# jinhojsk515/spmm

Hardware: AMD Instinct MI355X
Metric: pretrain molecules/sec (higher is better)
Workload: dtype bf16; 1 GPU; SPMM pretrain step, text 12 layers (fusion at 6) + PV 6 layers, H=768, 12 heads, queue 36864, train mode (dropout 0.1), fwd+bwd+clip+AdamW+EMA; global_batch=128, seq_len=128, parallelism=dp1, schedule=eager launches on three HIP streams, packed text rows

## Files before the change

include/spmm_hip.h:

```cpp
#ifndef SPMM_HIP_H
#define SPMM_HIP_H

#include <stdint.h>

#ifdef __HIPCC__
#include <hip/hip_runtime.h>
typedef hipStream_t spmm_stream_t;
#else
typedef void* spmm_stream_t;
#endif

#ifdef __cplusplus
extern "C" {
#endif

int spmm_version(void);
const char* spmm_last_error(void);

#define SPMM_EPI_BF16 0
#define SPMM_EPI_GELU 1
#define SPMM_EPI_F32 2
#define SPMM_EPI_F32_ATOMIC 3
#define SPMM_EPI_GELU_GRAD 4
#define SPMM_EPI_F32_ACC 5
#define SPMM_EPI_GELU_DERIV 6
#define SPMM_EPI_MUL 7

#define SPMM_GEMM_AUTO 0
#define SPMM_GEMM_K128 1
#define SPMM_GEMM_K256x128 2
#define SPMM_GEMM_K256 3
#define SPMM_GEMM_K128PC 5
#define SPMM_GEMM_K256P8 8
#define SPMM_GEMM_K256P8_TILES 9
#define SPMM_GEMM_AUTO_TILES 16
int spmm_gemm_nt(const void* A, long lda, const void* W, long ldw, int M, int N, int K, int splits, const float* bias,
                 const float* div_ptr, float alpha, const void* R, long ldr, const void* G, long ldg, void* C, long ldc,
                 void* C2, long ldc2, int epi, float* colsum, int kernel, const int* M_dev, spmm_stream_t stream);
long spmm_gemm_tn_workspace_bytes(int M, int N, int K, int splits);
int spmm_gemm_tn_splits(int M, int N, int K, int kernel);
int spmm_gemm_tn(const void* A, long lda, const void* B, long ldb, int M, int N, int K, int splits, float alpha, float* C,
                 long ldc, float* workspace, int kernel, const int* M_dev, spmm_stream_t stream);
int spmm_gemm_tn_reduce(const float* ws, int ns, int N, int K, float* C, long ldc, spmm_stream_t stream);
int spmm_colsum_bf16(const void* x, long ld, int R, int C, float* out, const int* R_dev, spmm_stream_t stream);

int spmm_attn_fwd(const void* Q, long ldq, const void* K, long ldk, const void* V, long ldv, const int* kmask,
                  const int* kv_seq, const int* q_row0, const int* q_len, const int* kv_row0, const int* kv_len, void* O,
                  long ldo, float* LSE, int nseq, int nH, int Lq, int Lkv, int causal_from, int is_cross, float dropout_p,
                  const uint64_t* seed_ptr, uint64_t seed_salt, int q_off, int kv_off, spmm_stream_t stream);
// ... 161 lines not shown
```

spmm_amd/csrc/gemm.hip:

```cpp
#include "common.h"
#include "../../include/spmm_hip.h"

namespace {

constexpr int BM = 128, BN = 128, BK = 64;
constexpr int TILE_BYTES = BM * BK * 2;
constexpr int STAGE_BYTES = 2 * TILE_BYTES;

enum Epi { EPI_BF16 = 0, EPI_GELU = 1, EPI_F32 = 2, EPI_F32_ATOMIC = 3, EPI_GELU_GRAD = 4, EPI_F32_ACC = 5, EPI_GELU_DERIV = 6, EPI_MUL = 7 };
constexpr bool epi_is_bf16(int e) { return e == EPI_BF16 || e == EPI_GELU || e == EPI_GELU_GRAD || e == EPI_GELU_DERIV || e == EPI_MUL; }

struct GemmP {
  const bf16* A; long lda;
  const bf16* W; long ldw;
  int M, N, K;
  int ksplit;
  const float* bias;
  const float* div_ptr;
  float alpha;
  const bf16* R; long ldr;
  const bf16* G; long ldg;
  void* C; long ldc;
  bf16* C2; long ldc2;
  float* colsum;
// ... 839 lines not shown
    if (p.colsum) {
#pragma unroll
      for (int e = 0; e < 8; ++e) {
        float t = cs[e];
        t += __shfl_xor(t, 8, 64);
        t += __shfl_xor(t, 16, 64);
        t += __shfl_xor(t, 32, 64);
        cs[e] = t;
      }
      if (lane < 8 && n_ok) {
#pragma unroll
        for (int e = 0; e < 8; ++e) atomicAdd(p.colsum + n + e, cs[e]);
      }
    }
  }
}

template <int EPI>
__global__ __launch_bounds__(512) void gemm_nt_p8_kernel(GemmP p) {
  extern __shared__ __attribute__((aligned(16))) char smem8[];
  const int tid = threadIdx.x, lane = tid & 63;
  const int wave = __builtin_amdgcn_readfirstlane(tid >> 6);
  const int wr = wave >> 2, wc = wave & 3;
  GEMM_DYN_M(p);
  const int ntm = (p.M + BM3 - 1) / BM3, ntn = (p.N + BN3 - 1) / BN3, nt = ntm * ntn;
  if ((int)blockIdx.x >= nt) return;
  const int nk = p.K / BK;

  f32x4 acc[2][4][4];
#define P8_ZERO()                                                              \
// ... 163 lines not shown
    P8_STAMP(2);

    if (wr == 0) P8_BAR();
    P8_SB();
    {
      int lane_e = lane;
      asm volatile("" : "+v"(lane_e));
      GemmP q = p;
      asm volatile("" : "+s"(q.C), "+s"(q.ldc), "+s"(q.C2), "+s"(q.ldc2));
      asm volatile("" : "+s"(q.R), "+s"(q.ldr), "+s"(q.G), "+s"(q.ldg));
      asm volatile("" : "+s"(q.bias), "+s"(q.colsum), "+s"(q.div_ptr), "+s"(q.alpha), "+s"(q.M), "+s"(q.N));
      auto hook = [](int) {};
      const uint32_t xb = lds0 + P8_LDS + wave * 4096;
      const int mb = cm0 + wr * 128, nb = cn0 + wc * 64;
      const bool interior = cm0 + BM3 <= q.M && cn0 + BN3 <= q.N;
      if constexpr (EPI == EPI_GELU_GRAD || EPI == EPI_MUL) {
        if (interior) p8_epilogue_blocks<EPI, true, true>(q, acc, xb, mb, nb, lane_e, hook);
        else p8_epilogue_blocks<EPI, false, true>(q, acc, xb, mb, nb, lane_e, hook);
      } else if (EPI == EPI_BF16 && q.R != nullptr) {
        if (interior) p8_epilogue_blocks<EPI, true, true>(q, acc, xb, mb, nb, lane_e, hook);
        else p8_epilogue_blocks<EPI, false, true>(q, acc, xb, mb, nb, lane_e, hook);
      } else {
        if (interior) p8_epilogue_blocks<EPI, true, false>(q, acc, xb, mb, nb, lane_e, hook);
        else p8_epilogue_blocks<EPI, false, false>(q, acc, xb, mb, nb, lane_e, hook);
      }
    }
    P8_SB();
    if (wr == 1) P8_BAR();
    P8_STAMP(4);
#ifdef P8_PROFILE
    ++prof_i;
// ... 20 lines not shown
#undef P8_LGKM0
}

template <typename K>
int raise_lds(K kernel, int bytes, const char* what) {
  hipError_t e = hipFuncSetAttribute((const void*)kernel, hipFuncAttributeMaxDynamicSharedMemorySize, bytes);
  if (e != hipSuccess) {
    spmm_set_error("spmm_gemm_nt: cannot raise the dynamic LDS of %s to %d: %s", what, bytes, hipGetErrorString(e));
    return SPMM_ERR_LAUNCH;
  }
  return SPMM_OK;
}

template <int EPI>
int launch_p8_one(const GemmP& p, hipStream_t st, bool persist) {
  static const int rc = raise_lds(gemm_nt_p8_kernel<EPI>, P8_LDS + P8_XLDS, "the 8-phase kernel");
  if (rc != SPMM_OK) return rc;
  const int nt = ((p.M + BM3 - 1) / BM3) * ((p.N + BN3 - 1) / BN3);
  static const int ncu = [] { int dev = 0, n = 0; (void)hipGetDevice(&dev); (void)hipDeviceGetAttribute(&n, hipDeviceAttributeMultiprocessorCount, dev); return n > 0 ? n & ~7 : 256; }();
  dim3 grid(persist && nt > ncu ? ncu : nt);
  hipLaunchKernelGGL((gemm_nt_p8_kernel<EPI>), grid, dim3(512), P8_LDS + P8_XLDS, st, p);
  return SPMM_OK;
}
int launch_p8(int epi, const GemmP& p, hipStream_t st, bool persist) {
  switch (epi) {
    case EPI_BF16: return launch_p8_one<EPI_BF16>(p, st, persist);
    case EPI_GELU: return launch_p8_one<EPI_GELU>(p, st, persist);
    case EPI_GELU_GRAD: return launch_p8_one<EPI_GELU_GRAD>(p, st, persist);
    case EPI_GELU_DERIV: return launch_p8_one<EPI_GELU_DERIV>(p, st, persist);
    case EPI_MUL: return launch_p8_one<EPI_MUL>(p, st, persist);
    default: return -1;
  }
}

template <int EPI>
int launch_v3_one(const GemmP& p, hipStream_t st) {
  static const int rc = raise_lds(gemm_nt_v3_kernel<EPI>, LDS3_BYTES, "the 256x256 kernel");
  if (rc != SPMM_OK) return rc;
  dim3 grid(((p.M + BM3 - 1) / BM3) * ((p.N + BN3 - 1) / BN3));
  hipLaunchKernelGGL((gemm_nt_v3_kernel<EPI>), grid, dim3(512), LDS3_BYTES, st, p);
  return SPMM_OK;
}
int launch_v3(int epi, const GemmP& p, hipStream_t st) {
  switch (epi) {
    case EPI_BF16: return launch_v3_one<EPI_BF16>(p, st);
// ... 51 lines not shown
    case EPI_BF16: hipLaunchKernelGGL((gemm_nt_kernel<EPI_BF16>), grid, dim3(256), 0, st, p); break;
    case EPI_GELU: hipLaunchKernelGGL((gemm_nt_kernel<EPI_GELU>), grid, dim3(256), 0, st, p); break;
    case EPI_F32: hipLaunchKernelGGL((gemm_nt_kernel<EPI_F32>), grid, dim3(256), 0, st, p); break;
    case EPI_F32_ATOMIC: hipLaunchKernelGGL((gemm_nt_kernel<EPI_F32_ATOMIC>), grid, dim3(256), 0, st, p); break;
    case EPI_GELU_GRAD: hipLaunchKernelGGL((gemm_nt_kernel<EPI_GELU_GRAD>), grid, dim3(256), 0, st, p); break;
    case EPI_F32_ACC: hipLaunchKernelGGL((gemm_nt_kernel<EPI_F32_ACC>), grid, dim3(256), 0, st, p); break;
    case EPI_GELU_DERIV: hipLaunchKernelGGL((gemm_nt_kernel<EPI_GELU_DERIV>), grid, dim3(256), 0, st, p); break;
    case EPI_MUL: hipLaunchKernelGGL((gemm_nt_kernel<EPI_MUL>), grid, dim3(256), 0, st, p); break;
    default: return -1;
  }
  return SPMM_OK;
}

inline bool is_bf16_epi(int epi) { return epi_is_bf16(epi); }
inline bool p8_ok(const GemmP& p, int epi) {
  return is_bf16_epi(epi) && p.K % 128 == 0 && p.N % 8 == 0 && (unsigned long)p.M * (unsigned long)p.lda * 2ul < (1ul << 32) &&
         (unsigned long)p.N * (unsigned long)p.ldw * 2ul < (1ul << 32);
}

int pick_tile(int M, int N, int epi) {
  const bool bf = is_bf16_epi(epi);
  if (M >= 6000) {
    const long t3 = (long)((M + 255) / 256) * ((N + 255) / 256);
    if (bf && t3 >= 96) return 3;
    return (epi != EPI_F32_ATOMIC) ? 2 : 1;
  }
  auto tiles = [&](int bm, int bn) { return (double)((M + bm - 1) / bm) * ((N + bn - 1) / bn); };
  auto fill = [](double t) { const double w = (double)(long)((t + 255) / 256); return t / (256.0 * w); };
  const double t3 = tiles(256, 256), t2 = tiles(256, 128), t1 = tiles(128, 128);
  const double s3 = bf ? 1.20 * fill(t3) : 0.0;
  const double s2 = (M >= 512 && epi != EPI_F32_ATOMIC) ? 0.85 * fill(t2) : 0.0;
  const double s1 = 0.80 * (t1 < 256 ? t1 / 256.0 : 1.0);
  if (s3 >= s2 && s3 >= s1) return 3;
  return s2 >= s1 ? 2 : 1;
}

}

extern "C" int spmm_gemm_nt(const void* A, long lda, const void* W, long ldw, int M, int N, int K, int splits,
// ... 13 lines not shown
  SPMM_CHECK_SHAPE(epi >= EPI_BF16 && epi <= EPI_MUL, "spmm_gemm_nt: unknown epilogue %d", epi);
  if (splits < 1) splits = 1;
  SPMM_CHECK_SHAPE(splits == 1 || epi == EPI_F32_ATOMIC, "spmm_gemm_nt: split-K needs the atomic epilogue");
  SPMM_CHECK_SHAPE((epi != EPI_GELU_GRAD && epi != EPI_MUL) || G != nullptr, "spmm_gemm_nt: the GELU-grad / multiply epilogues need G");
  SPMM_CHECK_SHAPE(colsum == nullptr || epi == EPI_BF16 || epi == EPI_GELU_GRAD || epi == EPI_MUL, "spmm_gemm_nt: colsum is only fused into the bf16 / GELU-grad / multiply epilogues");
  int ksplit = ((K / 64 + splits - 1) / splits) * 64;
  splits = (K + ksplit - 1) / ksplit;
  GemmP p;
  p.A = (const bf16*)A; p.lda = lda; p.W = (const bf16*)W; p.ldw = ldw;
  p.M = M; p.N = N; p.K = K; p.ksplit = ksplit; p.bias = bias; p.div_ptr = div_ptr; p.alpha = alpha;
  p.R = (const bf16*)R; p.ldr = ldr; p.G = (const bf16*)G; p.ldg = ldg; p.C = C; p.ldc = ldc;
  p.C2 = (bf16*)C2; p.ldc2 = ldc2; p.colsum = colsum;
  p.M_ptr = nullptr;
  p.order = K > 1024 ? 0 : 2;

  int k = kernel == SPMM_GEMM_AUTO_TILES ? 0 : kernel;
  if (k == 0) {
    const int tile = splits > 1 ? 1 : pick_tile(M, N, epi);
    k = tile == 3 ? (p8_ok(p, epi) ? (kernel == SPMM_GEMM_AUTO_TILES ? 9 : 8) : 3) : tile;
    if (k == 2 && (epi == EPI_F32_ATOMIC || M < 512)) k = 1;
  }
  const bool pc_fits = (unsigned long)p.M * (unsigned long)p.lda * 2ul < (1ul << 32) && (unsigned long)p.N * (unsigned long)p.ldw * 2ul < (1ul << 32);
  const long t128 = (long)((M + BM - 1) / BM) * ((N + BN - 1) / BN) * splits;
  if (k == 1 && kernel != 1 && pc_fits && PC_AUTO && t128 <= 256 && ksplit >= 4 * BK) k = 5;
  SPMM_CHECK_SHAPE(k == 1 || k == 2 || k == 3 || k == 5 || k == 8 || k == 9, "spmm_gemm_nt: unknown kernel selector %d", kernel);
  SPMM_CHECK_SHAPE(k != 5 || pc_fits, "spmm_gemm_nt: kernel 5 addresses its operands with 32-bit byte offsets (< 4 GiB each)");
  SPMM_CHECK_SHAPE((k != 8 && k != 9) || p8_ok(p, epi), "spmm_gemm_nt: the 8-phase kernel needs a bf16-output epilogue, K %% 128 == 0, N %% 8 == 0 and operands < 4 GiB");
  SPMM_CHECK_SHAPE(k != 3 || is_bf16_epi(epi), "spmm_gemm_nt: the 256x256 kernel has bf16-output epilogues only");
  SPMM_CHECK_SHAPE(k != 2 || epi != EPI_F32_ATOMIC, "spmm_gemm_nt: the 256x128 kernel has no atomic epilogue");
  SPMM_CHECK_SHAPE(k == 1 || k == 5 || splits == 1, "spmm_gemm_nt: split-K runs on the 128x128 kernels only");
  p.M_ptr = M_dev;
  int rc;
  if (k == 8 || k == 9) rc = launch_p8(epi, p, stream, k == 8);
  else if (k == 3) rc = launch_v3(epi, p, stream);
  else if (k == 2) rc = launch_v2(epi, p, stream);
  else if (k == 5) rc = launch_pc(epi, p, dim3(((M + BM - 1) / BM) * ((N + BN - 1) / BN), 1, splits), stream);
  else rc = launch_v1(epi, p, dim3(((M + BM - 1) / BM) * ((N + BN - 1) / BN), 1, splits), stream);
  if (rc > 0) return rc;
  if (rc < 0) { spmm_set_error("spmm_gemm_nt: epilogue %d is not built for kernel %d", epi, k); return SPMM_ERR_UNSUPPORTED; }
  SPMM_LAUNCH_CHECK("spmm_gemm_nt");
  return SPMM_OK;
}
// ... 1 lines not shown
```

spmm_amd/engine.py:

```python
from __future__ import annotations

import contextlib
import functools
from dataclasses import dataclass
from typing import List, NamedTuple, Optional

import numpy as np
import torch

from . import ops, streams
from .config import BertConfig, SPMMConfig
from .options import EngineOptions
from .params import ParamStore

BF = torch.bfloat16
LOSS_MLM, LOSS_MPM, LOSS_ITA, LOSS_ITM = 0, 1, 2, 3


def _ceil(x, m):
    return (x + m - 1) // m * m


class KVSource:

    def __init__(self, kv: torch.Tensor, U: int, Lkv: int, row0=None, length=None, pack_idx=None, proj=None):
        self.kv, self.U, self.Lkv, self.row0, self.len, self.pack_idx = kv, U, Lkv, row0, length, pack_idx
        self.proj = proj
        self._idx: List[torch.Tensor] = []
        self.nseq = 0
        self.start = self.list = None

    def add(self, idx: torch.Tensor) -> int:
        off = self.nseq
        self._idx.append(idx)
        self.nseq += idx.numel()
        return off

    def preset(self, nseq: int, start: torch.Tensor, lst: torch.Tensor):
        self.nseq, self.start, self.list = nseq, start, lst
        return self

    def finalize(self):
        idx = torch.cat(self._idx)
        order = torch.sort(idx, stable=True).indices
        start = torch.zeros(self.U + 1, dtype=torch.int32, device=idx.device)
        counts = torch.zeros(self.U, dtype=torch.int64, device=idx.device).index_add_(0, idx, torch.ones_like(idx))
        start[1:] = torch.cumsum(counts, 0)
        self.start, self.list = start, order.to(torch.int32)
        return self


@dataclass
class SelfKV:
    x: torch.Tensor
    dx: Optional[torch.Tensor] = None
    rows_dev: Optional[torch.Tensor] = None


@dataclass
class Group:
    row0: int
    nseq: int
    L: int
    kmask: Optional[torch.Tensor]
# ... 329 lines not shown
                   dxsum=P.g(op + "dense.bias"), rows_dev=md, beta_from_y=P.w(op + "LayerNorm.bias") if from_y else None)
        self._wgrad(dx, A, P.g(op + "dense.weight"), md=md)
        return dz, dx

    def _attn_block_fwd(self, pfx, c, X, groups, save, cross, X32=None, kv_tap=None, xattn_tap=None):
        P, H, nH = self.P, c.hidden_size, c.num_attention_heads
        salts_a = [self._next_salt() for _ in groups]
        salt_h = self._next_salt()
        sv = {"X": X, "salt_a": salts_a, "cross": cross}
        if not cross:
            ctx, core = self._self_attn_fwd(pfx, c, X, groups, save, salts_a, kv_tap)
        else:
            sv["Qc"] = Qc = ops.gemm_nt(X, P.wb(pfx + ".self.query.weight"), self._new(X.shape[0], H), bias=P.w(pfx + ".self.query.bias"),
                                        M_dev=groups.rows_dev)
            done = {id(g.src): g.src.proj[pfx] for g in groups if g.src is not None and g.src.proj and pfx in g.src.proj}
            kv_of = functools.partial(self._xattn_kv, P.fused(pfx + ".self.", ("key", "value"), "weight"),
                                      P.fused(pfx + ".self.", ("key", "value"), "bias", what="w"), done)
            if xattn_tap is not None:
                for gi, g in enumerate(groups):
                    xattn_tap(gi, g, Qc[g.rows], kv_of(g)[:, :H])
            fx = self.opt.fused_xattn
            fused = ((fx is True or fx == "all" or (fx == "nograd" and not save)) and not self._xattn_off and X32 is None
                     and groups.rows_dev is None and all(ops.xattn_supported(H, nH, g.L, g.Lkv) for g in groups))
            if fused:
                y, out = self._xattn_fused_fwd(pfx, c, X, Qc, kv_of, groups, save, salts_a, salt_h)
                g0 = groups.groups[0]
                if not self._xattn_checked and not ops._DRY_RUN and g0.row0 == 0:
                    self._xattn_checked = True
                    agrees, dmax, dmean = self._xattn_agrees(pfx, c, X, Qc, out["KV"][0], g0, y, salts_a[0], salt_h)
                    if not agrees:
                        import warnings
                        warnings.warn(f"spmm_amd: the fused cross-attention kernel disagrees with the composite launches (max |dy| {dmax:.3g}, "
# ... 29 lines not shown
                                                      M_dev=g.self_src.rows_dev)
                KVs = skv[id(g.self_src)]
                ops.attn_fwd_long(QKV[r, :H], KVs[:, :H], KVs[:, H:], ctx[r], lse, Lkv=g.skv_L, kmask=None, causal_from=g.nseq,
                                  kv_row0=g.skv_row0, kv_len=g.skv_len, **kw)
            else:
                ops.attn_fwd_long(QKV[r, :H], QKV[r, H:2 * H], QKV[r, 2 * H:], ctx[r], lse, Lkv=g.L, kmask=g.kmask, causal_from=g.causal_from,
                                  kv_row0=g.q_row0, kv_len=g.q_len, **kw)
            lses.append(lse)
        return ctx, dict(QKV=QKV, SKV=skv, lse=lses)

    def _xattn_kv(self, Wkv, bkv, done, g):
        key, kv = (id(g), g.kv) if g.src is None else (id(g.src), g.src.kv)
        if key not in done:
            done[key] = ops.gemm_nt(kv, Wkv, self._new(kv.shape[0], Wkv.shape[0]), bias=bkv)
        return done[key]

    def _xattn_core_fwd(self, c, Qc, kv_of, groups, save, salts):
        H, nH = c.hidden_size, c.num_attention_heads
        ctx, KVs, lses = self._new(Qc.shape[0], H), [], []
        for g, salt in zip(groups, salts):
            KV = kv_of(g)
            lse = self._new(g.nseq, nH, g.L, dtype=torch.float32) if save else None
            ops.attn_fwd_long(Qc[g.rows], KV[:, :H], KV[:, H:], ctx[g.rows], lse, nseq=g.nseq, nH=nH, Lq=g.L, Lkv=g.Lkv, is_cross=True,
                              dropout_p=self._p_attn(c), seed=self.seed, salt=salt, **g.cross_layout())
            KVs.append(KV)
            lses.append(lse)
        return ctx, dict(KV=KVs, lse=lses)

    def _xattn_fused_fwd(self, pfx, c, X, Qc, kv_of, groups, save, salts, salt_h):
        P, H, nH, M = self.P, c.hidden_size, c.num_attention_heads, X.shape[0]
# ... 56 lines not shown
                                  dQKV[r, H:2 * H], dQKV[r, 2 * H:], Lkv=g.L, kmask=g.kmask, causal_from=g.causal_from,
                                  kv_row0=g.q_row0, kv_len=g.q_len, **kw)
            self._wgrad(dQKV, X, gWqkv, gbqkv, md=md)
            WT = self._wT(pfx + ".self.qkv", P.fused(pfx + ".self.", ("query", "key", "value"), "weight", what="w"))
            for src, dKVs in dskv.values():
                self._wgrad(dKVs, src.x, gWqkv[H:], gbqkv[H:], md=src.rows_dev)
                ops.gemm_nt(dKVs, WT[:, H:], src.dx, M_dev=src.rows_dev)
            ops.gemm_nt(dQKV, WT, dX, R=dz, M_dev=md)
        else:
            Qc = sv["Qc"]
            dQc = self._new(M, H)
            gWkv = P.fused(pfx + ".self.", ("key", "value"), "weight", what="g")
            gbkv = P.fused(pfx + ".self.", ("key", "value"), "bias", what="g")
            WkvT = self._wT(pfx + ".self.kv", P.fused(pfx + ".self.", ("key", "value"), "weight", what="w"))
            pool = {}
            for i, g in enumerate(groups):
                r = g.rows
                KV = sv["KV"][i]
                src = g.src
                if src is not None:
                    if id(src) not in pool:
                        pool[id(src)] = (src, self._new(src.nseq * src.Lkv, 2 * H))
                    dKV = pool[id(src)][1][g.kv_off * g.Lkv:(g.kv_off + g.nseq) * g.Lkv]
                else:
                    dKV = self._new(g.nseq * g.Lkv, 2 * H)
                ops.attn_bwd_long(Qc[r], KV[:, :H], KV[:, H:], sv["ctx"][r], sv["lse"][i], dctx[r], dQc[r], dKV[:, :H], dKV[:, H:],
                                  nseq=g.nseq, nH=nH, Lq=g.L, Lkv=g.Lkv, is_cross=True, dropout_p=pa, seed=self.seed, salt=sv["salt_a"][i],
                                  **g.cross_layout())
                if src is None:
                    self._wgrad(dKV, g.kv, gWkv, gbkv)
                    ops.gemm_nt(dKV, WkvT, dkv_acc[i], epi=ops.EPI_F32_ACC)
            for src, dKV in pool.values():
                W = src.Lkv * 2 * H
                dKVu = ops.segment_sum_bf16(dKV.view(src.nseq, W), src.start, src.list, self._new(src.U, W)).view(-1, 2 * H)
                if src.pack_idx is not None:
                    dKVu = ops.gather_rows(self._new(src.pack_idx.numel(), 2 * H), dKVu, src.pack_idx)
                self._wgrad(dKVu, src.kv, gWkv, gbkv)
                ops.gemm_nt(dKVu, WkvT, dkv_acc[id(src)], epi=ops.EPI_F32_ACC)
            self._wgrad(dQc, X, P.g(pfx + ".self.query.weight"), P.g(pfx + ".self.query.bias"), md=md)
            ops.gemm_nt(dQc, self._wT(pfx + ".self.query", P.w(pfx + ".self.query.weight")), dX, R=dz, M_dev=md)
        return dX

    def _layer_fwd(self, lp, c, has_cross, X, groups, save, X32=None, kv_tap=None, xattn_tap=None):
        P, H, I, M = self.P, c.hidden_size, c.intermediate_size, X.shape[0]
        tap = {} if kv_tap is None else {"kv_tap": kv_tap}
        a, sv1, a32 = self._attn_block_fwd(lp + "attention", c, X, groups, save, cross=False, X32=X32, **tap)
        sv2 = None
        if has_cross:
            xtap = {} if xattn_tap is None else {"xattn_tap": xattn_tap}
            a, sv2, a32 = self._attn_block_fwd(lp + "crossattention", c, a, groups, save, cross=True, X32=a32, **xtap)
        h = self._new(M, I)
        dact = self._new(M, I) if save else None
        ops.gemm_nt(a, P.wb(lp + "intermediate.dense.weight"), h, bias=P.w(lp + "intermediate.dense.bias"),
# ... 157 lines not shown
```

spmm_amd/options.py:

```python
from __future__ import annotations

import dataclasses
import os
from dataclasses import dataclass

_ENV = {
    "pack_text": ("SPMM_PACK_TEXT", lambda s: s != "0"),
    "cls_only_top": ("SPMM_CLS_ONLY_TOP", lambda s: s != "0"),
    "multi_stream": ("SPMM_STREAMS", lambda s: s != "1"),
    "wgrad_stream": ("SPMM_WGRAD_STREAM", lambda s: s != "0"),
    "pv_wgrad_inline": ("SPMM_PV_WGRAD_INLINE", int),
    "ln_from_y": ("SPMM_LN_FROM_Y", lambda s: s != "0"),
    "resid_fp32": ("SPMM_RESID_FP32", lambda s: s == "1"),
    "fused_xattn": ("SPMM_FUSED_XATTN", lambda s: {"0": "off", "1": "all"}.get(s, s)),
    "grad_overlap": ("SPMM_GRAD_OVERLAP", lambda s: s != "0"),
    "grad_wire": ("SPMM_GRAD_WIRE", str),
    "nt_under_comm": ("SPMM_NT_UNDER_COMM", str),
    "force_dist": ("SPMM_FORCE_DIST", lambda s: s == "1"),
    "dp_four_streams": ("SPMM_DP_FOUR_STREAMS", lambda s: s != "0"),
    "probe_streams": ("SPMM_PROBE_STREAMS", lambda s: s != "0"),
    "schedule_check": ("SPMM_SCHEDULE_CHECK", lambda s: s != "0"),
}


@dataclass
class EngineOptions:
    pack_text: bool = True
    cls_only_top: bool = True
    multi_stream: bool = True
    wgrad_stream: bool = True
    pv_wgrad_inline: int = 4
    ln_from_y: bool = True
    fused_xattn: str = "nograd"
    resid_fp32: bool = False
    grad_overlap: bool = True
    grad_wire: str = "fp32"
    nt_under_comm: str = "auto"
    force_dist: bool = False
    dp_four_streams: bool = True
    schedule_check: bool = True
    probe_streams: bool = False

    @classmethod
    def from_env(cls, **overrides) -> "EngineOptions":
        kw = {}
        for field, (var, parse) in _ENV.items():
            if var in os.environ:
# ... 18 lines not shown
```

spmm_amd/step.py:

```python
from __future__ import annotations

from typing import Callable, Optional, Tuple

import torch

from . import ops, streams
from .engine import STREAM_TOKENS_MAX, BF, LOSS_ITA, LOSS_ITM, LOSS_MLM, LOSS_MPM, Batch, Engine, Group, KVSource, SelfKV, _ceil


class PretrainStep(Engine):
    def _s6_forward_cls(self, B, Lt, M, pk, mask32, neg, y1, y2, prop_embeds, text_embeds, save):
        cfg = self.cfg
        ct = cfg.text
        H, Lp, f, n = ct.hidden_size, cfg.n_props + 1, ct.fusion_layer, ct.num_hidden_layers
        fp = ops.fusion_plan(neg, pk, Lp)
        o_tp = 3 * B * Lp
        o_lm = o_tp + 2 * M
        o_12 = o_lm + B * Lt
        o_8 = o_12 + B * Lp
        Rcap = fp["Rcap"]
        X6 = ops.gather_rows2(self._new(Rcap, H), y1, fp["idx6"], y2)
        src_pv = KVSource(prop_embeds.view(B * Lp, H), B, Lp).preset(4 * B, fp["start_p"], fp["list_p"])
        src_text = KVSource(text_embeds, B, Lt, row0=pk["row0"], length=pk["len"], pack_idx=pk["rows"]).preset(4 * B, fp["start_t"], fp["list_t"])
        ar = fp["ar"]
        g_lo = Batch([Group(0, 3 * B, Lp, None, 3 * B).bind(src_text, fp["kvidx_pv"], 0),
                      Group(o_tp, 2 * B, Lt, None, 2 * B, q_row0=fp["qrow0_tp"], q_len=fp["qlen_tp"], nrows=2 * M).bind(src_pv, fp["kvidx_tp"], 0),
                      Group(o_lm, B, Lt, mask32, 0).bind(src_pv, ar, 2 * B),
                      Group(o_12, B, Lp, None, 0).bind(src_text, ar, 3 * B),
                      Group(o_8, B, Lt, None, B, q_row0=fp["row0_8"], q_len=fp["len_8"], nrows=B * Lt).bind(src_pv, ar, 3 * B)],
                     rows_dev=fp["rows_dev"])
        y, tape_lo, _ = self.stack_fwd("text_encoder.bert.", ct, range(f, n - 1), True, X6, g_lo, save)
        ntop = 6 * B + B * Lt + B * Lp
        Xtop = ops.gather_rows2(self._new(ntop, H), y, fp["idx_top"])
        skv_a = SelfKV(y[:o_lm])
        skv_b = SelfKV(y[o_8:], rows_dev=fp["mn_dev"])
        g_top = Batch([Group(0, 3 * B, 1, None, 3 * B, self_src=skv_a, skv_row0=fp["skv_row0_pv"], skv_len=fp["skv_len_pv"], skv_L=Lp).bind(src_text, fp["kvidx_pv"], 0),
                       Group(3 * B, 2 * B, 1, None, 2 * B, self_src=skv_a, skv_row0=fp["skv_row0_tx"], skv_len=fp["skv_len_tx"], skv_L=Lt).bind(src_pv, fp["kvidx_tp"], 0),
                       Group(5 * B, B, 1, None, B, self_src=skv_b, skv_row0=fp["row0_8"], skv_len=fp["len_8"], skv_L=Lt).bind(src_pv, ar, 3 * B),
                       Group(6 * B, B, Lt, mask32, 0).bind(src_pv, ar, 2 * B),
                       Group(6 * B + B * Lt, B, Lp, None, 0).bind(src_text, ar, 3 * B)])
        ytop, sv_top, _ = self._layer_fwd(f"text_encoder.bert.encoder.layer.{n - 1}.", ct, True, Xtop, g_top, save)
        return dict(fp=fp, ytop=ytop, sv_top=sv_top, g_top=g_top, skv=(skv_a, skv_b), g_lo=g_lo, tape_lo=tape_lo, src_text=src_text, src_pv=src_pv,
                    o_tp=o_tp, o_lm=o_lm, o_12=o_12, o_8=o_8, ntop=ntop, Rcap=Rcap)

    def _s6_backward_cls(self, T, dYtop, d_pe, d_te):
        S6, B, Lt, M = T["S6"], T["B"], T["Lt"], T["M"]
        cfg = self.cfg
        ct = cfg.text
        H, Lp, f, n = ct.hidden_size, cfg.n_props + 1, ct.fusion_layer, ct.num_hidden_layers
        fp, o_lm, o_8 = S6["fp"], S6["o_lm"], S6["o_8"]
        dkv_acc = {id(S6["src_text"]): d_te[:M], id(S6["src_pv"]): d_pe.view(B * Lp, H)}
        dX6 = self._new(S6["Rcap"], H)
        S6["skv"][0].dx = dX6[:o_lm]
        S6["skv"][1].dx = dX6[o_8:]
        dXtop = self._layer_bwd(f"text_encoder.bert.encoder.layer.{n - 1}.", ct, S6["sv_top"], dYtop, S6["g_top"], dkv_acc)
        if self.layer_done_cb is not None:
            self._layer_done(f"text_encoder.bert.encoder.layer.{n - 1}.")
        ops.add_rows_bf16(dX6, fp["idx_top"][:6 * B], dXtop[:6 * B])
        dX6[o_lm:o_8].copy_(dXtop[6 * B:])
        return self.stack_bwd("text_encoder.bert.", ct, range(f, n - 1), S6["tape_lo"], dX6, S6["g_lo"], dkv_acc=dkv_acc)

    def forward(self, prop: torch.Tensor, ids: torch.Tensor, mask: torch.Tensor, *, mpm_mask: Optional[torch.Tensor] = None,
                neg_idx: Optional[Tuple[torch.Tensor, torch.Tensor]] = None, gather: Optional[Callable] = None,
                save: bool = True, aux: Optional[dict] = None, n_tokens: Optional[int] = None) -> torch.Tensor:
        cfg, P = self.cfg, self.P
        ct, cp = cfg.text, cfg.prop
# ... 171 lines not shown
            else:
                src_text = KVSource(text_embeds, B, Lt)
                te = text_embeds.view(B, Lt * H)
                te_neg = ops.gather_rows(self._new(B, Lt * H), te, neg[B:])
                qtext = torch.cat([te, te, te_neg, hidden10.view(B, Lt * H)]).view(4 * B * Lt, H)
                if r32:
                    te32 = text_embeds_32.view(B, Lt * H)
                    qtext_32 = torch.cat([te32, te32, te32.index_select(0, neg[B:]), hidden10_32.view(B, Lt * H)]).view(4 * B * Lt, H)
                kvmask_qpv = torch.cat([mask32, mask32, mask_neg, mask32])
                gt = [Group(4 * B * Lp, 4 * B, Lt, kvmask_qpv, 3 * B).attend(src_pv, torch.cat([ar, neg[:B], ar, ar]))]
                neg_rows, cls_text, Mn = None, torch.arange(3 * B, dtype=torch.int64, device=self.dev) * Lt, B * Lt
            X6 = torch.cat([qpv, qtext])
            g6 = Batch([Group(0, 4 * B, Lp, None, 3 * B, kv_mask=kvmask_qpv).attend(src_text, torch.cat([ar, ar, neg[B:], ar]))] + gt)
            src_text.finalize()
            src_pv.finalize()
            y6, tape6, y6_32 = self.stack_fwd("text_encoder.bert.", ct, range(f, n), True, X6, g6, save, X32=torch.cat([qpv_32, qtext_32]) if r32 else None)
            ypv, ytext = y6[:4 * B * Lp], y6[4 * B * Lp:]
            ypv_h, ytext_h = (y6_32[:4 * B * Lp], y6_32[4 * B * Lp:]) if r32 else (ypv, ytext)

            vl_logits = self._new(3 * B, 2, dtype=torch.float32) if aux is not None else None
            itm_text = ytext_h.index_select(0, cls_text)
            ops.itm_head(ypv_h, Lp * H, itm_text, H, H, P.w("itm_head.weight"), P.w("itm_head.bias"), n=3 * B, B=B, losses=self.losses,
                         slot=LOSS_ITM, logits=vl_logits)

        feat_pm, feat_tm = feats["property_proj_m"][0], feats["text_proj_m"][0]
        if gather is not None:
            g = gather(torch.cat([feat_pm, feat_tm, self.nan_flag.to(torch.float32).expand(B, 1)], 1))
            feat_pm, feat_tm = g[:, :E].contiguous(), g[:, E:2 * E].contiguous()
            self.nan_flag.copy_((g[:, 2 * E].abs().sum() > 0).to(torch.int32).view(1))
        ptr = P.buffers["queue_ptr"]
# ... 50 lines not shown

        dmln = self._new(B * Lp, H)
        ops.mpm_head(T["mpmsv"].ln.y, Lp, H, P.w("property_mtr_head.3.weight"), P.w("property_mtr_head.3.bias"), T["prop"], T["mpm_mask"], B=B,
                     ws=self.icount[4:8], losses=scratch, slot=LOSS_MPM, dh=dmln, dw=P.g("property_mtr_head.3.weight"),
                     db=P.g("property_mtr_head.3.bias"), gscale=gs[1:2])
        dmpre = self._transform_bwd(T["mpmsv"], dmln)
        ops.gemm_nt(dmpre, self._wT("property_mtr_head.0", P.w("property_mtr_head.0.weight")), dY_mpm)

        V = ct.vocab_size
        dlogits = self._new(B * Lt, _ceil(V, 64))
        ops.lm_loss(T["logits"], T["logits_m"], T["ids32"], nseq=B, L=Lt, V=V, alpha=self.alpha, ws=self.icount[0:4], losses=scratch,
                    slot=LOSS_MLM, dlogits=dlogits, gscale=gs[0:1])
        self.lm_head_bwd("text_encoder.", ct, T["lmsv"], dlogits, out=dY_lm)

        neg_p, neg_t = T["neg"][:B], T["neg"][B:]
        d_pe = self._zeros(B, Lp * H, dtype=torch.float32)
        d_te = self._zeros(M + 1, H, dtype=torch.float32)
        if S6 is not None:
            ytop = S6["ytop"]
            ops.itm_head(ytop[:3 * B], H, ytop[3 * B:6 * B], H, H, P.w("itm_head.weight"), P.w("itm_head.bias"), n=3 * B, B=B, losses=scratch,
                         slot=LOSS_ITM, dxa=dYtop[:3 * B], dxb=dYtop[3 * B:6 * B], dW=P.g("itm_head.weight"), db=P.g("itm_head.bias"), gscale=gs[3:4])
            dX6 = self._s6_backward_cls(T, dYtop, d_pe, d_te)
            dXpv = dX6[:3 * B * Lp].view(3 * B, Lp * H)
            dXt = dX6[S6["o_tp"]:S6["o_lm"]]
            ops.acc_rows(d_pe, dXpv[0:B])
            ops.acc_rows(d_pe, dXpv[B:2 * B], idx=neg_p, atomic=True)
            ops.acc_rows(d_pe, dXpv[2 * B:3 * B])
            ops.acc_rows(d_te[:M], dXt[:M])
            ops.acc_rows(d_te[:M], dXt[M:2 * M])
            ops.acc_rows(d_te, dX6[S6["o_8"]:], idx=S6["fp"]["neg_rows"], atomic=True)
            dXt_lm, dX12 = dX6[S6["o_lm"]:S6["o_12"]], dX6[S6["o_12"]:S6["o_8"]]
        else:
            ditm = self._new(3 * B, H)
            ops.itm_head(T["ypv"], Lp * H, T["itm_text"], H, H, P.w("itm_head.weight"), P.w("itm_head.bias"), n=3 * B, B=B, losses=scratch,
                         slot=LOSS_ITM, dxa=dYpv, dxb=ditm, dW=P.g("itm_head.weight"), db=P.g("itm_head.bias"), gscale=gs[3:4])
            dYtext.index_copy_(0, T["cls_text"], ditm)
            dX6 = self.stack_bwd("text_encoder.bert.", ct, range(f, n), T["tape6"], dY6, T["g6"],
                                 dkv_acc={id(T["src_text"]): d_te[:M], id(T["src_pv"]): d_pe.view(B * Lp, H)})
            dXpv, dXt = dX6[:4 * B * Lp].view(4 * B, Lp * H), dX6[4 * B * Lp:]
            ops.acc_rows(d_pe, dXpv[0:B])
            ops.acc_rows(d_pe, dXpv[B:2 * B], idx=neg_p, atomic=True)
            ops.acc_rows(d_pe, dXpv[2 * B:3 * B])
            if pk:
                ops.acc_rows(d_te[:M], dXt[:M])
                ops.acc_rows(d_te[:M], dXt[M:2 * M])
                nr = T["neg_rows"]
                ops.acc_rows(d_te, dXt[2 * M:2 * M + T["Mn"]], idx=torch.where(nr < M, nr, torch.full_like(nr, -1)), atomic=True)
            else:
                dte, dxt = d_te[:M].view(B, Lt * H), dXt.view(4 * B, Lt * H)
                ops.acc_rows(dte, dxt[0:B])
                ops.acc_rows(dte, dxt[B:2 * B])
                ops.acc_rows(dte, dxt[2 * B:3 * B], idx=neg_t, atomic=True)
            dXt_lm, dX12 = dXt[nt6 - B * Lt:], dXpv[3 * B:].reshape(B * Lp, H)
# ... 47 lines not shown
```

Measured before the change: 2455 molecules/s.

## Add joint cross-attention KV projection and 8-phase f32-accumulate GEMM epilogue

Adds an EPI_F32_ACC epilogue to the 8-phase 256x256 GEMM kernel that reads, adds and writes fp32 output directly, and lets auto selection route large f32-accumulate GEMMs to it instead of the 256x128 kernel. It also adds an optional joint KV mode that concatenates property and text embeddings into one buffer, so cross-attention K/V projections and their backward dgrad/wgrad run as one GEMM instead of two. The joint mode is off by default and costs an extra concat copy plus a shared fp32 accumulator. The new epilogue adds read-modify-write traffic in the persistent kernel.

```diff
diff --git a/include/spmm_hip.h b/include/spmm_hip.h
--- a/include/spmm_hip.h
+++ b/include/spmm_hip.h
@@ -33,6 +33,8 @@
 #define SPMM_GEMM_K128PC 5
 #define SPMM_GEMM_K256P8 8
 #define SPMM_GEMM_K256P8_TILES 9
+#define SPMM_GEMM_K256P8_ACC 10
+#define SPMM_GEMM_K256P8_ACC_TILES 11
 #define SPMM_GEMM_AUTO_TILES 16
 int spmm_gemm_nt(const void* A, long lda, const void* W, long ldw, int M, int N, int K, int splits, const float* bias,
                  const float* div_ptr, float alpha, const void* R, long ldr, const void* G, long ldg, void* C, long ldc,
diff --git a/spmm_amd/csrc/gemm.hip b/spmm_amd/csrc/gemm.hip
--- a/spmm_amd/csrc/gemm.hip
+++ b/spmm_amd/csrc/gemm.hip
@@ -877,6 +877,73 @@
       }
     }
   }
+}
+
+template <bool INTERIOR>
+__device__ __forceinline__ void p8_epilogue_f32_acc(const GemmP& p, f32x4 (&acc)[2][4][4], int m_base, int n_base, int lane) {
+  float scale = p.alpha;
+  if (p.div_ptr) scale /= *p.div_ptr;
+  const int m = lane & 15, g = lane >> 4;
+  const long row0 = m_base + m;
+  const int n0 = n_base + 4 * g;
+  GLOBAL_AS float* const C = (GLOBAL_AS float*)p.C;
+  const GLOBAL_AS float* const bias = (const GLOBAL_AS float*)p.bias;
+  const GLOBAL_AS bf16* const R = (const GLOBAL_AS bf16*)p.R;
+  f32x4 b[4];
+  bool n_ok[4];
+  long nn[4];
+#pragma unroll
+  for (int ni = 0; ni < 4; ++ni) {
+    n_ok[ni] = INTERIOR || n0 + ni * 16 < p.N;
+    nn[ni] = n_ok[ni] ? n0 + ni * 16 : 0;
+    b[ni] = f32x4{0.f, 0.f, 0.f, 0.f};
+  }
+  if (p.bias) {
+#pragma unroll
+    for (int ni = 0; ni < 4; ++ni) b[ni] = *(const GLOBAL_AS f32x4*)(bias + nn[ni]);
+  }
+  f32x4 c[2][4];
+#define P8_ACC_LOAD(BLK)                                                                                 \
+  do {                                                                                                   \
+    long r_ = row0 + (BLK) * 16;                                                                         \
+    if (!INTERIOR) r_ = r_ < p.M ? r_ : p.M - 1;                                                         \
+    _Pragma("unroll") for (int ni = 0; ni < 4; ++ni) c[(BLK) & 1][ni] = *(const GLOBAL_AS f32x4*)(C + r_ * p.ldc + nn[ni]); \
+  } while (0)
+  P8_ACC_LOAD(0);
+#pragma unroll
+  for (int h = 0; h < 2; ++h)
+#pragma unroll
+    for (int mi = 0; mi < 4; ++mi) {
+      const int blk = h * 4 + mi;
+      const long row = row0 + blk * 16;
+      const bool m_ok = INTERIOR || row < p.M;
+      if (blk < 7) P8_ACC_LOAD(blk + 1);
+      f32x4 v[4];
+#pragma unroll
+      for (int ni = 0; ni < 4; ++ni)
+#pragma unroll
+        for (int j = 0; j < 4; ++j) v[ni][j] = acc[h][mi][ni][j] * scale + b[ni][j];
+#pragma unroll
+      for (int ni = 0; ni < 4; ++ni) acc[h][mi][ni] = f32x4{0.f, 0.f, 0.f, 0.f};
+      if (p.R) {
+        const long rr = INTERIOR ? row : (m_ok ? row : (long)p.M - 1);
+#pragma unroll
+        for (int ni = 0; ni < 4; ++ni) {
+          const bf16x4 r = *(const GLOBAL_AS bf16x4*)(R + rr * p.ldr + nn[ni]);
+#pragma unroll
+          for (int j = 0; j < 4; ++j) v[ni][j] += (float)r[j];
+        }
+      }
+#pragma unroll
+      for (int ni = 0; ni < 4; ++ni) {
+        f32x4 o = c[blk & 1][ni];
+#pragma unroll
+        for (int j = 0; j < 4; ++j) o[j] += v[ni][j];
+        if constexpr (!INTERIOR) asm volatile("" : "+v"(o));
+        if (m_ok && n_ok[ni]) *(GLOBAL_AS f32x4*)(C + row * p.ldc + nn[ni]) = o;
+      }
+    }
+#undef P8_ACC_LOAD
 }
 
 template <int EPI>
@@ -1070,7 +1137,10 @@
       const uint32_t xb = lds0 + P8_LDS + wave * 4096;
       const int mb = cm0 + wr * 128, nb = cn0 + wc * 64;
       const bool interior = cm0 + BM3 <= q.M && cn0 + BN3 <= q.N;
-      if constexpr (EPI == EPI_GELU_GRAD || EPI == EPI_MUL) {
+      if constexpr (EPI == EPI_F32_ACC) {
+        if (interior) p8_epilogue_f32_acc<true>(q, acc, mb, nb, lane_e);
+        else p8_epilogue_f32_acc<false>(q, acc, mb, nb, lane_e);
+      } else if constexpr (EPI == EPI_GELU_GRAD || EPI == EPI_MUL) {
         if (interior) p8_epilogue_blocks<EPI, true, true>(q, acc, xb, mb, nb, lane_e, hook);
         else p8_epilogue_blocks<EPI, false, true>(q, acc, xb, mb, nb, lane_e, hook);
       } else if (EPI == EPI_BF16 && q.R != nullptr) {
@@ -1121,12 +1191,13 @@
 
 template <int EPI>
 int launch_p8_one(const GemmP& p, hipStream_t st, bool persist) {
-  static const int rc = raise_lds(gemm_nt_p8_kernel<EPI>, P8_LDS + P8_XLDS, "the 8-phase kernel");
+  constexpr int lds = EPI == EPI_F32_ACC ? P8_LDS : P8_LDS + P8_XLDS;
+  static const int rc = raise_lds(gemm_nt_p8_kernel<EPI>, lds, "the 8-phase kernel");
   if (rc != SPMM_OK) return rc;
   const int nt = ((p.M + BM3 - 1) / BM3) * ((p.N + BN3 - 1) / BN3);
   static const int ncu = [] { int dev = 0, n = 0; (void)hipGetDevice(&dev); (void)hipDeviceGetAttribute(&n, hipDeviceAttributeMultiprocessorCount, dev); return n > 0 ? n & ~7 : 256; }();
   dim3 grid(persist && nt > ncu ? ncu : nt);
-  hipLaunchKernelGGL((gemm_nt_p8_kernel<EPI>), grid, dim3(512), P8_LDS + P8_XLDS, st, p);
+  hipLaunchKernelGGL((gemm_nt_p8_kernel<EPI>), grid, dim3(512), lds, st, p);
   return SPMM_OK;
 }
 int launch_p8(int epi, const GemmP& p, hipStream_t st, bool persist) {
@@ -1136,6 +1207,7 @@
     case EPI_GELU_GRAD: return launch_p8_one<EPI_GELU_GRAD>(p, st, persist);
     case EPI_GELU_DERIV: return launch_p8_one<EPI_GELU_DERIV>(p, st, persist);
     case EPI_MUL: return launch_p8_one<EPI_MUL>(p, st, persist);
+    case EPI_F32_ACC: return launch_p8_one<EPI_F32_ACC>(p, st, persist);
     default: return -1;
   }
 }
@@ -1217,7 +1289,7 @@
 
 inline bool is_bf16_epi(int epi) { return epi_is_bf16(epi); }
 inline bool p8_ok(const GemmP& p, int epi) {
-  return is_bf16_epi(epi) && p.K % 128 == 0 && p.N % 8 == 0 && (unsigned long)p.M * (unsigned long)p.lda * 2ul < (1ul << 32) &&
+  return (is_bf16_epi(epi) || epi == EPI_F32_ACC) && p.K % 128 == 0 && p.N % 8 == 0 && (unsigned long)p.M * (unsigned long)p.lda * 2ul < (1ul << 32) &&
          (unsigned long)p.N * (unsigned long)p.ldw * 2ul < (1ul << 32);
 }
 
@@ -1225,7 +1297,7 @@
   const bool bf = is_bf16_epi(epi);
   if (M >= 6000) {
     const long t3 = (long)((M + 255) / 256) * ((N + 255) / 256);
-    if (bf && t3 >= 96) return 3;
+    if ((bf || epi == EPI_F32_ACC) && t3 >= 96) return 3;
     return (epi != EPI_F32_ATOMIC) ? 2 : 1;
   }
   auto tiles = [&](int bm, int bn) { return (double)((M + bm - 1) / bm) * ((N + bn - 1) / bn); };
@@ -1269,10 +1341,14 @@
   p.M_ptr = nullptr;
   p.order = K > 1024 ? 0 : 2;
 
-  int k = kernel == SPMM_GEMM_AUTO_TILES ? 0 : kernel;
+  const bool p8_acc = kernel == SPMM_GEMM_K256P8_ACC || kernel == SPMM_GEMM_K256P8_ACC_TILES;
+  SPMM_CHECK_SHAPE(!p8_acc || (epi == EPI_F32_ACC && p8_ok(p, epi)),
+                   "spmm_gemm_nt: selectors 10 / 11 run EPI_F32_ACC on the 8-phase kernel: K %% 128 == 0, N %% 8 == 0 and operands < 4 GiB");
+  const bool forced_p8 = kernel == SPMM_GEMM_K256P8 || kernel == SPMM_GEMM_K256P8_TILES;
+  int k = kernel == SPMM_GEMM_AUTO_TILES ? 0 : (p8_acc ? kernel - 2 : kernel);
   if (k == 0) {
     const int tile = splits > 1 ? 1 : pick_tile(M, N, epi);
-    k = tile == 3 ? (p8_ok(p, epi) ? (kernel == SPMM_GEMM_AUTO_TILES ? 9 : 8) : 3) : tile;
+    k = tile == 3 ? (p8_ok(p, epi) ? (kernel == SPMM_GEMM_AUTO_TILES ? 9 : 8) : (is_bf16_epi(epi) ? 3 : 2)) : tile;
     if (k == 2 && (epi == EPI_F32_ATOMIC || M < 512)) k = 1;
   }
   const bool pc_fits = (unsigned long)p.M * (unsigned long)p.lda * 2ul < (1ul << 32) && (unsigned long)p.N * (unsigned long)p.ldw * 2ul < (1ul << 32);
@@ -1280,7 +1356,7 @@
   if (k == 1 && kernel != 1 && pc_fits && PC_AUTO && t128 <= 256 && ksplit >= 4 * BK) k = 5;
   SPMM_CHECK_SHAPE(k == 1 || k == 2 || k == 3 || k == 5 || k == 8 || k == 9, "spmm_gemm_nt: unknown kernel selector %d", kernel);
   SPMM_CHECK_SHAPE(k != 5 || pc_fits, "spmm_gemm_nt: kernel 5 addresses its operands with 32-bit byte offsets (< 4 GiB each)");
-  SPMM_CHECK_SHAPE((k != 8 && k != 9) || p8_ok(p, epi), "spmm_gemm_nt: the 8-phase kernel needs a bf16-output epilogue, K %% 128 == 0, N %% 8 == 0 and operands < 4 GiB");
+  SPMM_CHECK_SHAPE((k != 8 && k != 9) || (p8_ok(p, epi) && (!forced_p8 || is_bf16_epi(epi))), "spmm_gemm_nt: the 8-phase kernel needs a bf16-output epilogue, K %% 128 == 0, N %% 8 == 0 and operands < 4 GiB");
   SPMM_CHECK_SHAPE(k != 3 || is_bf16_epi(epi), "spmm_gemm_nt: the 256x256 kernel has bf16-output epilogues only");
   SPMM_CHECK_SHAPE(k != 2 || epi != EPI_F32_ATOMIC, "spmm_gemm_nt: the 256x128 kernel has no atomic epilogue");
   SPMM_CHECK_SHAPE(k == 1 || k == 5 || splits == 1, "spmm_gemm_nt: split-K runs on the 128x128 kernels only");
diff --git a/spmm_amd/engine.py b/spmm_amd/engine.py
--- a/spmm_amd/engine.py
+++ b/spmm_amd/engine.py
@@ -29,6 +29,8 @@
         self._idx: List[torch.Tensor] = []
         self.nseq = 0
         self.start = self.list = None
+        self.joint: Optional["JointKV"] = None
+        self.joint_row0 = 0
 
     def add(self, idx: torch.Tensor) -> int:
         off = self.nseq
@@ -48,6 +50,17 @@
         start[1:] = torch.cumsum(counts, 0)
         self.start, self.list = start, order.to(torch.int32)
         return self
+
+
+class JointKV:
+
+    def __init__(self, sources, new):
+        rows = [s.kv.shape[0] for s in sources]
+        self.kv = torch.cat([s.kv for s in sources], out=new(sum(rows), sources[0].kv.shape[1]))
+        self.sources, r0 = list(sources), 0
+        for s, n in zip(sources, rows):
+            s.kv, s.joint, s.joint_row0 = self.kv[r0:r0 + n], self, r0
+            r0 += n
 
 
 @dataclass
@@ -407,8 +420,10 @@
             sv["Qc"] = Qc = ops.gemm_nt(X, P.wb(pfx + ".self.query.weight"), self._new(X.shape[0], H), bias=P.w(pfx + ".self.query.bias"),
                                         M_dev=groups.rows_dev)
             done = {id(g.src): g.src.proj[pfx] for g in groups if g.src is not None and g.src.proj and pfx in g.src.proj}
-            kv_of = functools.partial(self._xattn_kv, P.fused(pfx + ".self.", ("key", "value"), "weight"),
-                                      P.fused(pfx + ".self.", ("key", "value"), "bias", what="w"), done)
+            Wkv, bkv = P.fused(pfx + ".self.", ("key", "value"), "weight"), P.fused(pfx + ".self.", ("key", "value"), "bias", what="w")
+            kv_of = functools.partial(self._xattn_kv, Wkv, bkv, done)
+            if self.opt.joint_kv:
+                self._xattn_kv_joint(Wkv, bkv, done, groups)
             if xattn_tap is not None:
                 for gi, g in enumerate(groups):
                     xattn_tap(gi, g, Qc[g.rows], kv_of(g)[:, :H])
@@ -468,6 +483,21 @@
         if key not in done:
             done[key] = ops.gemm_nt(kv, Wkv, self._new(kv.shape[0], Wkv.shape[0]), bias=bkv)
         return done[key]
+
+    @staticmethod
+    def _joints_of(groups, skip=()):
+        seen, joints = {}, {}
+        for g in groups:
+            if g.src is not None and g.src.joint is not None and id(g.src) not in skip:
+                seen[id(g.src)] = g.src
+                joints[id(g.src.joint)] = g.src.joint
+        return [J for J in joints.values() if len(J.sources) > 1 and all(id(s) in seen for s in J.sources)]
+
+    def _xattn_kv_joint(self, Wkv, bkv, done, groups):
+        for J in self._joints_of(groups, done):
+            KVj = ops.gemm_nt(J.kv, Wkv, self._new(J.kv.shape[0], Wkv.shape[0]), bias=bkv)
+            for s in J.sources:
+                done[id(s)] = KVj[s.joint_row0:s.joint_row0 + s.kv.shape[0]]
 
     def _xattn_core_fwd(self, c, Qc, kv_of, groups, save, salts):
         H, nH = c.hidden_size, c.num_attention_heads
@@ -554,6 +584,7 @@
             gbkv = P.fused(pfx + ".self.", ("key", "value"), "bias", what="g")
             WkvT = self._wT(pfx + ".self.kv", P.fused(pfx + ".self.", ("key", "value"), "weight", what="w"))
             pool = {}
+            joint = {id(J): (J, self._new(J.kv.shape[0], 2 * H)) for J in (self._joints_of(groups) if self.opt.joint_kv else ()) if id(J) in dkv_acc}
             for i, g in enumerate(groups):
                 r = g.rows
                 KV = sv["KV"][i]
@@ -572,11 +603,17 @@
                     ops.gemm_nt(dKV, WkvT, dkv_acc[i], epi=ops.EPI_F32_ACC)
             for src, dKV in pool.values():
                 W = src.Lkv * 2 * H
-                dKVu = ops.segment_sum_bf16(dKV.view(src.nseq, W), src.start, src.list, self._new(src.U, W)).view(-1, 2 * H)
+                out = joint[id(src.joint)][1][src.joint_row0:src.joint_row0 + src.kv.shape[0]] if id(src.joint) in joint else None
+                dense = out is not None and src.pack_idx is None
+                dKVu = ops.segment_sum_bf16(dKV.view(src.nseq, W), src.start, src.list, out.view(src.U, W) if dense else self._new(src.U, W)).view(-1, 2 * H)
                 if src.pack_idx is not None:
-                    dKVu = ops.gather_rows(self._new(src.pack_idx.numel(), 2 * H), dKVu, src.pack_idx)
-                self._wgrad(dKVu, src.kv, gWkv, gbkv)
-                ops.gemm_nt(dKVu, WkvT, dkv_acc[id(src)], epi=ops.EPI_F32_ACC)
+                    dKVu = ops.gather_rows(self._new(src.pack_idx.numel(), 2 * H) if out is None else out, dKVu, src.pack_idx)
+                if out is None:
+                    self._wgrad(dKVu, src.kv, gWkv, gbkv)
+                    ops.gemm_nt(dKVu, WkvT, dkv_acc[id(src)], epi=ops.EPI_F32_ACC)
+            for J, dKVj in joint.values():
+                self._wgrad(dKVj, J.kv, gWkv, gbkv)
+                ops.gemm_nt(dKVj, WkvT, dkv_acc[id(J)], epi=ops.EPI_F32_ACC)
             self._wgrad(dQc, X, P.g(pfx + ".self.query.weight"), P.g(pfx + ".self.query.bias"), md=md)
             ops.gemm_nt(dQc, self._wT(pfx + ".self.query", P.w(pfx + ".self.query.weight")), dX, R=dz, M_dev=md)
         return dX
diff --git a/spmm_amd/options.py b/spmm_amd/options.py
--- a/spmm_amd/options.py
+++ b/spmm_amd/options.py
@@ -12,6 +12,7 @@
     "pv_wgrad_inline": ("SPMM_PV_WGRAD_INLINE", int),
     "ln_from_y": ("SPMM_LN_FROM_Y", lambda s: s != "0"),
     "resid_fp32": ("SPMM_RESID_FP32", lambda s: s == "1"),
+    "joint_kv": ("SPMM_JOINT_KV", lambda s: s != "0"),
     "fused_xattn": ("SPMM_FUSED_XATTN", lambda s: {"0": "off", "1": "all"}.get(s, s)),
     "grad_overlap": ("SPMM_GRAD_OVERLAP", lambda s: s != "0"),
     "grad_wire": ("SPMM_GRAD_WIRE", str),
@@ -31,6 +32,7 @@
     wgrad_stream: bool = True
     pv_wgrad_inline: int = 4
     ln_from_y: bool = True
+    joint_kv: bool = False
     fused_xattn: str = "nograd"
     resid_fp32: bool = False
     grad_overlap: bool = True
diff --git a/spmm_amd/step.py b/spmm_amd/step.py
--- a/spmm_amd/step.py
+++ b/spmm_amd/step.py
@@ -5,7 +5,7 @@
 import torch
 
 from . import ops, streams
-from .engine import STREAM_TOKENS_MAX, BF, LOSS_ITA, LOSS_ITM, LOSS_MLM, LOSS_MPM, Batch, Engine, Group, KVSource, SelfKV, _ceil
+from .engine import STREAM_TOKENS_MAX, BF, LOSS_ITA, LOSS_ITM, LOSS_MLM, LOSS_MPM, Batch, Engine, Group, JointKV, KVSource, SelfKV, _ceil
 
 
 class PretrainStep(Engine):
@@ -22,6 +22,7 @@
         X6 = ops.gather_rows2(self._new(Rcap, H), y1, fp["idx6"], y2)
         src_pv = KVSource(prop_embeds.view(B * Lp, H), B, Lp).preset(4 * B, fp["start_p"], fp["list_p"])
         src_text = KVSource(text_embeds, B, Lt, row0=pk["row0"], length=pk["len"], pack_idx=pk["rows"]).preset(4 * B, fp["start_t"], fp["list_t"])
+        self._joint_sources(src_pv, src_text)
         ar = fp["ar"]
         g_lo = Batch([Group(0, 3 * B, Lp, None, 3 * B).bind(src_text, fp["kvidx_pv"], 0),
                       Group(o_tp, 2 * B, Lt, None, 2 * B, q_row0=fp["qrow0_tp"], q_len=fp["qlen_tp"], nrows=2 * M).bind(src_pv, fp["kvidx_tp"], 0),
@@ -43,13 +44,25 @@
         return dict(fp=fp, ytop=ytop, sv_top=sv_top, g_top=g_top, skv=(skv_a, skv_b), g_lo=g_lo, tape_lo=tape_lo, src_text=src_text, src_pv=src_pv,
                     o_tp=o_tp, o_lm=o_lm, o_12=o_12, o_8=o_8, ntop=ntop, Rcap=Rcap)
 
-    def _s6_backward_cls(self, T, dYtop, d_pe, d_te):
+    def _joint_sources(self, src_pv: KVSource, src_text: KVSource):
+        return JointKV([src_pv, src_text], self._new) if self.opt.joint_kv else None
+
+    def _hub_grads(self, B, Lp, H, M, src_pv, src_text):
+        J = src_pv.joint
+        if J is not None and J is src_text.joint and self.opt.joint_kv:
+            acc = self._zeros(B * Lp + M + 1, H, dtype=torch.float32)
+            d_pe, d_te = acc[:B * Lp].view(B, Lp * H), acc[B * Lp:]
+            return d_pe, d_te, {id(J): acc[:B * Lp + M], id(src_text): d_te[:M], id(src_pv): d_pe.view(B * Lp, H)}
+        d_pe = self._zeros(B, Lp * H, dtype=torch.float32)
+        d_te = self._zeros(M + 1, H, dtype=torch.float32)
+        return d_pe, d_te, {id(src_text): d_te[:M], id(src_pv): d_pe.view(B * Lp, H)}
+
+    def _s6_backward_cls(self, T, dYtop, dkv_acc):
         S6, B, Lt, M = T["S6"], T["B"], T["Lt"], T["M"]
         cfg = self.cfg
         ct = cfg.text
         H, Lp, f, n = ct.hidden_size, cfg.n_props + 1, ct.fusion_layer, ct.num_hidden_layers
         fp, o_lm, o_8 = S6["fp"], S6["o_lm"], S6["o_8"]
-        dkv_acc = {id(S6["src_text"]): d_te[:M], id(S6["src_pv"]): d_pe.view(B * Lp, H)}
         dX6 = self._new(S6["Rcap"], H)
         S6["skv"][0].dx = dX6[:o_lm]
         S6["skv"][1].dx = dX6[o_8:]
@@ -251,6 +264,7 @@
             g6 = Batch([Group(0, 4 * B, Lp, None, 3 * B, kv_mask=kvmask_qpv).attend(src_text, torch.cat([ar, ar, neg[B:], ar]))] + gt)
             src_text.finalize()
             src_pv.finalize()
+            self._joint_sources(src_pv, src_text)
             y6, tape6, y6_32 = self.stack_fwd("text_encoder.bert.", ct, range(f, n), True, X6, g6, save, X32=torch.cat([qpv_32, qtext_32]) if r32 else None)
             ypv, ytext = y6[:4 * B * Lp], y6[4 * B * Lp:]
             ypv_h, ytext_h = (y6_32[:4 * B * Lp], y6_32[4 * B * Lp:]) if r32 else (ypv, ytext)
@@ -331,13 +345,12 @@
         self.lm_head_bwd("text_encoder.", ct, T["lmsv"], dlogits, out=dY_lm)
 
         neg_p, neg_t = T["neg"][:B], T["neg"][B:]
-        d_pe = self._zeros(B, Lp * H, dtype=torch.float32)
-        d_te = self._zeros(M + 1, H, dtype=torch.float32)
+        d_pe, d_te, dkv_acc = self._hub_grads(B, Lp, H, M, *((S6["src_pv"], S6["src_text"]) if S6 is not None else (T["src_pv"], T["src_text"])))
         if S6 is not None:
             ytop = S6["ytop"]
             ops.itm_head(ytop[:3 * B], H, ytop[3 * B:6 * B], H, H, P.w("itm_head.weight"), P.w("itm_head.bias"), n=3 * B, B=B, losses=scratch,
                          slot=LOSS_ITM, dxa=dYtop[:3 * B], dxb=dYtop[3 * B:6 * B], dW=P.g("itm_head.weight"), db=P.g("itm_head.bias"), gscale=gs[3:4])
-            dX6 = self._s6_backward_cls(T, dYtop, d_pe, d_te)
+            dX6 = self._s6_backward_cls(T, dYtop, dkv_acc)
             dXpv = dX6[:3 * B * Lp].view(3 * B, Lp * H)
             dXt = dX6[S6["o_tp"]:S6["o_lm"]]
             ops.acc_rows(d_pe, dXpv[0:B])
@@ -352,8 +365,7 @@
             ops.itm_head(T["ypv"], Lp * H, T["itm_text"], H, H, P.w("itm_head.weight"), P.w("itm_head.bias"), n=3 * B, B=B, losses=scratch,
                          slot=LOSS_ITM, dxa=dYpv, dxb=ditm, dW=P.g("itm_head.weight"), db=P.g("itm_head.bias"), gscale=gs[3:4])
             dYtext.index_copy_(0, T["cls_text"], ditm)
-            dX6 = self.stack_bwd("text_encoder.bert.", ct, range(f, n), T["tape6"], dY6, T["g6"],
-                                 dkv_acc={id(T["src_text"]): d_te[:M], id(T["src_pv"]): d_pe.view(B * Lp, H)})
+            dX6 = self.stack_bwd("text_encoder.bert.", ct, range(f, n), T["tape6"], dY6, T["g6"], dkv_acc=dkv_acc)
             dXpv, dXt = dX6[:4 * B * Lp].view(4 * B, Lp * H), dX6[4 * B * Lp:]
             ops.acc_rows(d_pe, dXpv[0:B])
             ops.acc_rows(d_pe, dXpv[B:2 * B], idx=neg_p, atomic=True)
```

Result: no change. 2461 molecules/s, median of 6 (+0.2%).
